# DomhnallBoyle/lip2speech-unit

Hardware: AMD Instinct MI355X
Metric: real-time factor (audio-sec/wall-sec), end-to-end lip->16kHz audio, 4s@25fps clips (higher is better)
Workload: dtype fp16; 1 GPU; e2e lip->units->wav (BASELINE configs[3]: AV-HuBERT large 24L + conformer 12x512 + multi_input HiFi-GAN), 4-s 100-frame 88x88 clips, batch 640 per GPU; clips_per_gpu=640, streams=1, clips_per_launch=640, frames_per_clip=100, hipgraph=True, input=uint8 96x96 frames resident in HBM, crop+normalise on device, enc_layers=24, conf_layers=12, parallelism=clip-parallel dp1

## Files before the change

lip2speech_unit_amd/csrc/phasegemm.hip:

```cpp
#include "l2s_common.h"
#include "tapgemm_tiles.h"
#include <cstdlib>

int l2s_phasegemm_f16_m0(const l2s_gemm_desc& d, hipStream_t st);
int l2s_phasegemm_f16_m1(const l2s_gemm_desc& d, hipStream_t st);
int l2s_phasegemm_f16_m2(const l2s_gemm_desc& d, hipStream_t st);
int l2s_phasegemm_bf16_m0(const l2s_gemm_desc& d, hipStream_t st);
int l2s_phasegemm_bf16_m1(const l2s_gemm_desc& d, hipStream_t st);
int l2s_phasegemm_bf16_m2(const l2s_gemm_desc& d, hipStream_t st);
int l2s_phasegemm_f16_m3(const l2s_gemm_desc& d, hipStream_t st);
int l2s_phasegemm_bf16_m3(const l2s_gemm_desc& d, hipStream_t st);

int l2s_phasegemm_ktab_launch(const l2s_gemm_desc& d, hipStream_t st) {
  if (d.mode != L2S_MODE_LINEAR || d.groups < 1) return L2S_EINVAL;
  const int fam = l2s::pick_epilogue(d.flags, d.act);
  if (fam != 2 && fam != l2s::L2S_EPI_G16A) return L2S_EUNSUPPORTED;
  if ((d.Cin % 64) || d.N < 256 || d.M < 256 || (d.M & 7) || (d.N & 7) || (d.lda & 7) || (d.ldc & 7) || (d.c_gstride & 63) ||
      (d.ldr & 7) || d.out_row_mul != 1 || d.out_row_add != 0)
    return L2S_EUNSUPPORTED;
  return d.dtype == L2S_F16 ? l2s_phasegemm_f16_m3(d, st) : l2s_phasegemm_bf16_m3(d, st);
}

bool l2s_phasegemm_eligible(const l2s_gemm_desc& d) {
  static const int mode = [] { const char* e = getenv("L2S_PHASEGEMM"); return e ? atoi(e) : 1; }();
  if (mode == 0) return false;
  if (d.groups > 1 || d.mode < 0 || d.mode > 2 || d.ktab) return false;
  if (d.mode == L2S_MODE_LINEAR && d.ntaps != 1) return false;
  if (d.mode == L2S_MODE_CONV1D && (d.T_out <= 0 || d.T_in <= 0)) return false;
  if (d.mode == L2S_MODE_CONV2D && (d.Ho <= 0 || d.Wo <= 0 || d.KW <= 0 || d.ntaps % d.KW)) return false;
  const int fam = l2s::pick_epilogue(d.flags, d.act);
  if (fam == l2s::L2S_EPI_ALL && !(l2s::is_x32(d.flags, d.act) && !(d.ldc & 3) && !(d.ldr & 3) && !(d.ldc2 & 3))) return false;
  static const int res_on = [] { const char* e = getenv("L2S_PHASEGEMM_RES"); return e ? atoi(e) : 1; }();
  if (!res_on && (fam == l2s::L2S_EPI_G16A || fam == l2s::L2S_EPI_G16B)) return false;
  if (fam == l2s::L2S_EPI_S32 && ((d.ldc & 3) || (d.ldr & 3))) return false;
  if ((d.Cin % 64) || d.N < 256 || d.M < 256 || (d.lda & 7)) return false;
  if (d.mode == L2S_MODE_LINEAR && ((d.M & 7) || (d.N & 7))) return false;
  if (mode == 2) return true;
  auto cdivl = [](long a, long b) { return (a + b - 1) / b; };
  const long tm = cdivl(d.M, 256);
  const long rounds_big = cdivl(tm * cdivl(d.N, 256), 256);
  if (rounds_big * ((long)d.Cin * d.ntaps / 64) < 20) return false;
  const double big = (double)rounds_big * 2.0 / 1.2;
  const double reg = (double)cdivl(tm * cdivl(d.N, 128), 256);
  return big < reg;
}

#ifdef L2S_WITH_WIDEGEMM
int l2s_widegemm_f16(const l2s_gemm_desc& d, hipStream_t st);
int l2s_widegemm_bf16(const l2s_gemm_desc& d, hipStream_t st);
static bool wide_ok(const l2s_gemm_desc& d) {
  static const int mode = [] { const char* e = getenv("L2S_WIDEGEMM"); return e ? atoi(e) : 0; }();
  if (mode == 0 || d.mode != L2S_MODE_LINEAR) return false;
  const int fam = l2s::pick_epilogue(d.flags, d.act);
  if (fam > l2s::L2S_EPI_G16A && fam != l2s::L2S_EPI_S32) return false;
  return !(d.M & 7) && !(d.N & 7);
}
#endif

int l2s_phasegemm_launch(const l2s_gemm_desc& d, hipStream_t st) {
  const bool h = d.dtype == L2S_F16;
#ifdef L2S_WITH_WIDEGEMM
  if (wide_ok(d)) return h ? l2s_widegemm_f16(d, st) : l2s_widegemm_bf16(d, st);
#endif
  switch (d.mode) {
    case L2S_MODE_LINEAR: return h ? l2s_phasegemm_f16_m0(d, st) : l2s_phasegemm_bf16_m0(d, st);
    case L2S_MODE_CONV1D: return h ? l2s_phasegemm_f16_m1(d, st) : l2s_phasegemm_bf16_m1(d, st);
    case L2S_MODE_CONV2D: return h ? l2s_phasegemm_f16_m2(d, st) : l2s_phasegemm_bf16_m2(d, st);
    default: return L2S_EINVAL;
  }
}
```

lip2speech_unit_amd/csrc/phasegemm_inst.hip:

```cpp
#include "phasegemm_kernel.h"

#define L2S_PCAT_(a, b) a##b
#define L2S_PCAT(a, b) L2S_PCAT_(a, b)
#if L2S_INST_ET == 0
using InstET = ElemF16;
#define L2S_INST_NAME L2S_PCAT(l2s_phasegemm_f16_m, L2S_INST_MODE)
#else
using InstET = ElemBF16;
#define L2S_INST_NAME L2S_PCAT(l2s_phasegemm_bf16_m, L2S_INST_MODE)
#endif

int L2S_INST_NAME(const l2s_gemm_desc& d, hipStream_t st) { return launch_phase_mode<InstET, L2S_INST_MODE>(d, st); }

#if defined(L2S_PHASE_STAMPS) && L2S_INST_ET == 0 && L2S_INST_MODE == 0
extern "C" int l2s_debug_phase_stamps(void* buf) { return phase_set_stamps(buf); }
#endif
```

lip2speech_unit_amd/csrc/phasegemm_kernel.h:

```cpp
#pragma once
#include "tapgemm_common.h"
#include <cstdlib>

using namespace l2s;

namespace {

constexpr int PBM = 256, PBN = 256, PBK = 64;
constexpr int Q_B = 128 * PBK * 2;
constexpr bool p_generic(int epi) { return epi == L2S_EPI_G16A || epi == L2S_EPI_G16B; }
constexpr int p_scr_b(int epi) { return p_generic(epi) ? 16 * 64 * 4 : 16 * (4 * 32 + 16); }
constexpr int p_smem(int epi) { return 8 * Q_B + 8 * p_scr_b(epi); }

#ifdef L2S_PHASE_STAMPS
__device__ unsigned long long* g_phase_stamps = nullptr;
#define PHSTAMP(i) { const unsigned long long now_ = __builtin_amdgcn_s_memtime(); ph_acc[i] += now_ - ph_last; ph_last = now_; }
#else
#define PHSTAMP(i)
#endif

constexpr int PG_KTAB = 3;
template <typename ET, int MODE_T, int EPI>
__global__ __launch_bounds__(512) void phasegemm_kernel(const l2s_gemm_desc p, const int tilesM, const int tilesN,
                                                        const int chunk, const int band) {
  constexpr bool KT = MODE_T == PG_KTAB;
  constexpr int MODE = KT ? (int)L2S_MODE_LINEAR : MODE_T;
  constexpr int MI = 8, NI = 4;
#ifdef L2S_NO_PAIRED
  constexpr bool PAIRED = false;
#else
  constexpr bool PAIRED = EPI <= L2S_EPI_G16A;
#endif
  extern __shared__ __attribute__((aligned(16))) uint16_t lds[];
  const int tid = threadIdx.x, lane = tid & 63;
  const int wave = __builtin_amdgcn_readfirstlane(tid >> 6);
  const int wr = wave >> 2, wc = wave & 3;
  const int K = p.Cin * p.ntaps;
  const int nk = K / PBK;
  const uint16_t* zero = reinterpret_cast<const uint16_t*>(&g_zero16);

  const int tiles_mn = tilesM * tilesN;
  const int ntiles = tiles_mn * (KT ? p.groups : 1);
  const int slot = blockIdx.x >> 3, slots = gridDim.x >> 3;
  const int lo = (blockIdx.x & 7) * chunk;
  const int hi = lo + chunk < ntiles ? lo + chunk : ntiles;
  const int my_n = (lo + slot < hi) ? (hi - lo - slot + slots - 1) / slots : 0;
  if (my_n == 0) return;
  const int total_q = my_n * nk * 4;
  auto tile_coords = [&](int i, int& m0, int& n0, int& g) {
    int l = lo + slot + i * slots;
    g = 0;
    if constexpr (KT) {
      const int per_m = p.groups * tilesN;
      const int mt = l / per_m, r = l - mt * per_m;
      g = r / tilesN;
      m0 = mt * PBM;
      n0 = (r - g * tilesN) * PBN;
      return;
    }
    const int bsz = band * tilesN;
    const int bi = l / bsz, idx = l - bi * bsz;
    const int rows = tilesM - bi * band < band ? tilesM - bi * band : band;
    const int tn = idx / rows;
    m0 = (bi * band + idx - tn * rows) * PBM;
    n0 = tn * PBN;
  };

  const int srow = lane >> 3;
  const int schunk = (lane & 7) ^ (srow & 7);
  const uint16_t* qa_ptr[2][2];
  int qa_t[2][2], qa_x[2][2];
  const uint16_t* qb_ptr[2][2];
  int run_tap = 0, run_c = 0, run_ky = 0, run_kx = 0;
  const char* sa_base[2][2] = {{nullptr, nullptr}, {nullptr, nullptr}};
  const char* sw_base[2][2] = {{nullptr, nullptr}, {nullptr, nullptr}};
  uint32_t a_lane = 0, w_lane[2] = {0, 0};
  if constexpr (MODE == L2S_MODE_LINEAR) {
    a_lane = (uint32_t)(srow * p.lda * 2 + (schunk << 4));
#pragma unroll
    for (int j = 0; j < 2; ++j) {
      const int within = 16 * (wave & 1) + 8 * j + srow;
      const int bchunk = PAIRED ? ((lane & 7) ^ paired_w_key(within)) : schunk;
      w_lane[j] = (uint32_t)(srow * K * 2 + (bchunk << 4));
    }
  }
  typedef const int32_t __attribute__((address_space(4)))* ktab_ptr_t;
  constexpr int KTN = L2S_KTAB_MAX;
  const ktab_ptr_t kt_tab = (ktab_ptr_t)(uintptr_t)p.ktab;
  ktab_ptr_t kt_row = kt_tab;
  int nk_stage = nk, kt_blk = 0, kt_win = 0;
  uint32_t kt_cur_a = 0, kt_cur_w = 0, kt_nxt_a = 0, kt_nxt_w = 0;
  const int kpb = KT ? p.Cin / PBK : 1;
  auto setup_issue = [&](int i) {
    int m0, n0, tg;
    tile_coords(i, m0, n0, tg);
    if constexpr (KT) {
      kt_row = kt_tab + tg * (2 + 2 * KTN);
      nk_stage = kt_row[0] * kpb;
      kt_blk = 0; kt_win = 0;
      kt_cur_a = (uint32_t)kt_row[2] * 2u; kt_cur_w = (uint32_t)kt_row[2 + KTN] * 2u;
      kt_nxt_a = (uint32_t)kt_row[3] * 2u; kt_nxt_w = (uint32_t)kt_row[3 + KTN] * 2u;
    }
#ifdef L2S_ABL_SAMETILE
    m0 = 0; n0 = 0;
#endif
    if constexpr (MODE == L2S_MODE_LINEAR) {
#pragma unroll
      for (int h = 0; h < 2; ++h)
#pragma unroll
        for (int j = 0; j < 2; ++j) {
          int mg = m0 + (wave >> 2) * 128 + h * 64 + 16 * (wave & 3) + 8 * j;
          mg = mg < p.M ? mg : p.M - 8;
          sa_base[h][j] = (const char*)p.A + (int64_t)mg * p.lda * 2;
          int ng = n0 + (wave >> 1) * 64 + h * 32 + 16 * (wave & 1) + 8 * j;
          ng = ng < p.N ? ng : p.N - 8;
          sw_base[h][j] = (const char*)p.W + (int64_t)ng * K * 2;
        }
      return;
    }
#pragma unroll
    for (int h = 0; h < 2; ++h)
#pragma unroll
      for (int j = 0; j < 2; ++j) {
        int m = m0 + (wave >> 2) * 128 + h * 64 + 16 * (wave & 3) + 8 * j + srow;
        m = m < p.M ? m : p.M - 1;
        qa_t[h][j] = 0; qa_x[h][j] = 0;
        if (MODE == L2S_MODE_LINEAR) {
          qa_ptr[h][j] = (const uint16_t*)p.A + (int64_t)m * p.lda + schunk * 8;
        } else if (MODE == L2S_MODE_CONV1D) {
          const int b = m / p.T_out, t = m - b * p.T_out;
          qa_ptr[h][j] = (const uint16_t*)p.A + (int64_t)b * p.T_in * p.lda + schunk * 8;
          qa_t[h][j] = t * p.stride + p.off;
        } else {
          const int hw = p.Ho * p.Wo;
          const int img = m / hw, rem = m - img * hw;
          const int oy = rem / p.Wo, ox = rem - oy * p.Wo;
          qa_ptr[h][j] = (const uint16_t*)p.A + (int64_t)img * p.Hi * p.Wi * p.lda + schunk * 8;
          qa_t[h][j] = oy * p.stride - p.pad;
          qa_x[h][j] = ox * p.stride - p.pad;
        }
        const int within = 16 * (wave & 1) + 8 * j + srow;
        int n = n0 + (wave >> 1) * 64 + h * 32 + within;
        n = n < p.N ? n : p.N - 1;
        const int bchunk = PAIRED ? ((lane & 7) ^ paired_w_key(within)) : schunk;
        qb_ptr[h][j] = (const uint16_t*)p.W + (int64_t)n * K + bchunk * 8;
      }
  };
  auto slot_off = [&](int b, int e) -> uint32_t { return (uint32_t)((b * 4 + e) * Q_B); };
  int s_i = 0, s_kt = 0, s_e = 0, s_par = 0, staged = 0;
  auto stage_one = [&](auto e_tag) {
    constexpr int E = decltype(e_tag)::value;
    const bool live = staged < total_q;
    const int k0 = s_kt * PBK;
    const int se = E >= 0 ? E : s_e;
    uint16_t* dst = lds + (slot_off(s_par, se) >> 1) + wave * 1024;
    const bool is_a = (se == 0) || (se == 3);
    const int h = (se == 2 || se == 3) ? 1 : 0;
    if constexpr (MODE == L2S_MODE_LINEAR) {
      static_assert(E >= 0, "LINEAR stages with a compile-time element");
      const uint32_t kb = (uint32_t)k0 * 2u;
      const uint32_t kba = KT ? kt_cur_a : kb, kbw = KT ? kt_cur_w : kb;
#pragma unroll
      for (int j = 0; j < 2; ++j) {
        const char* g = is_a ? sa_base[h][j] + (size_t)kba + (size_t)a_lane : sw_base[h][j] + (size_t)kbw + (size_t)w_lane[j];
#ifdef L2S_ABL_ZEROSRC
        g = (const char*)zero;
#endif
#if defined(L2S_ABL_WARMDMA)
        if (staged < 8) __builtin_amdgcn_global_load_lds((gptr_t)g, (lptr_t)(dst + j * 512), 16, 0, 0);
#elif !defined(L2S_ABL_NODMA)
        __builtin_amdgcn_global_load_lds((gptr_t)g, (lptr_t)(dst + j * 512), 16, 0, 0);
#endif
      }
      return;
    }
#pragma unroll
    for (int j = 0; j < 2; ++j) {
      const uint16_t* g;
      bool ok = live;
      if (!is_a) {
        g = qb_ptr[h][j] + k0;
      } else if (MODE == L2S_MODE_LINEAR) {
        g = qa_ptr[h][j] + k0;
      } else if (MODE == L2S_MODE_CONV1D) {
        const int st = qa_t[h][j] + run_tap * p.dil;
        ok = ok && ((unsigned)st < (unsigned)p.T_in);
        g = qa_ptr[h][j] + (st * p.lda + run_c);
      } else {
        const int iy = qa_t[h][j] + run_ky, ix = qa_x[h][j] + run_kx;
        ok = ok && ((unsigned)iy < (unsigned)p.Hi) && ((unsigned)ix < (unsigned)p.Wi);
        g = qa_ptr[h][j] + ((iy * p.Wi + ix) * p.lda + run_c);
      }
      g = ok ? g : zero;
#ifdef L2S_ABL_ZEROSRC
      g = zero;
#endif
#ifndef L2S_ABL_NODMA
      __builtin_amdgcn_global_load_lds((gptr_t)g, (lptr_t)(dst + j * 512), 16, 0, 0);
#endif
    }
  };
  auto stage_advance = [&]() {
    const bool live = staged < total_q;
    ++staged;
    if constexpr (MODE == L2S_MODE_LINEAR) {
      if (++s_e == 4) {
        s_e = 0;
        s_par ^= 1;
        if constexpr (KT) {
          if (!(s_i + 1 == my_n && s_kt + 1 == nk_stage)) {
            if (++s_kt == nk_stage) {
              s_kt = 0;
              setup_issue(++s_i);
            } else if (++kt_win == kpb) {
              kt_win = 0;
              ++kt_blk;
              kt_cur_a = kt_nxt_a; kt_cur_w = kt_nxt_w;
              const int nb = kt_blk + 1 < KTN ? kt_blk + 1 : KTN - 1;
              kt_nxt_a = (uint32_t)kt_row[2 + nb] * 2u; kt_nxt_w = (uint32_t)kt_row[2 + KTN + nb] * 2u;
            } else {
              kt_cur_a += PBK * 2; kt_cur_w += PBK * 2;
            }
          }
        } else if (staged < total_q && ++s_kt == nk) {
          s_kt = 0;
          setup_issue(++s_i);
        }
      }
      return;
    }
    if (++s_e == 4) {
      s_e = 0;
      s_par ^= 1;
      if (MODE != L2S_MODE_LINEAR) {
        run_c += PBK;
        if (run_c >= p.Cin) {
          run_c = 0;
          ++run_tap;
          if (++run_kx == p.KW) { run_kx = 0; ++run_ky; }
        }
      }
      if (live && ++s_kt == nk) {
        s_kt = 0;
        run_tap = 0; run_c = 0; run_ky = 0; run_kx = 0;
        if (++s_i < my_n) setup_issue(s_i);
      }
    }
  };

  const int lm = lane & 15, lg = lane >> 4;
  const uint32_t lds_base = (uint32_t)(uintptr_t)(lptr_t)lds;
  const uint32_t k0_off = (uint32_t)(lm * 128 + (((0 + lg) ^ (lm & 7)) << 4));
  const uint32_t k1_off = (uint32_t)(lm * 128 + (((4 + lg) ^ (lm & 7)) << 4));
  const uint32_t a_row = (uint32_t)(wr * 64) * 128;
  const uint32_t b_row = (uint32_t)(wc * 32) * 128;
  frag16 fa[4][2], fb[2][2][2];
  auto read_a = [&](uint32_t qbase) {
    const uint32_t a0 = qbase + a_row + k0_off, a1 = qbase + a_row + k1_off;
    lds_read_b128<0>(fa[0][0], a0); lds_read_b128<2048>(fa[1][0], a0); lds_read_b128<4096>(fa[2][0], a0); lds_read_b128<6144>(fa[3][0], a0);
    lds_read_b128<0>(fa[0][1], a1); lds_read_b128<2048>(fa[1][1], a1); lds_read_b128<4096>(fa[2][1], a1); lds_read_b128<6144>(fa[3][1], a1);
  };
  uint32_t bk_off[2][2];
#pragma unroll
  for (int s2 = 0; s2 < 2; ++s2)
#pragma unroll
    for (int ks = 0; ks < 2; ++ks)
      bk_off[s2][ks] = PAIRED ? paired_w_off(lm, s2, 4 * ks + lg) : (uint32_t)(s2 * 2048) + (ks ? k1_off : k0_off);
  auto read_b = [&](frag16(&f)[2][2], uint32_t qbase) {
    const uint32_t b = qbase + b_row;
    lds_read_b128<0>(f[0][0], b + bk_off[0][0]); lds_read_b128<0>(f[1][0], b + bk_off[1][0]);
    lds_read_b128<0>(f[0][1], b + bk_off[0][1]); lds_read_b128<0>(f[1][1], b + bk_off[1][1]);
  };

  f32x4_t acc[MI][NI];
#pragma unroll
  for (int i = 0; i < MI; ++i)
#pragma unroll
    for (int j = 0; j < NI; ++j) acc[i][j] = f32x4_t{0.f, 0.f, 0.f, 0.f};

  setup_issue(0);
  stage_one(std::integral_constant<int, 0>{}); stage_advance();
  stage_one(std::integral_constant<int, 1>{}); stage_advance();
  stage_one(std::integral_constant<int, 2>{}); stage_advance();
  stage_one(std::integral_constant<int, 3>{}); stage_advance();
  stage_one(std::integral_constant<int, 0>{}); stage_advance();
  stage_one(std::integral_constant<int, 1>{}); stage_advance();
  wait_vmcnt<8>();
  __builtin_amdgcn_s_barrier();
  if (wr == 1) __builtin_amdgcn_s_barrier();

  auto phase = [&](auto q_tag, const int par) {
    constexpr int Q = decltype(q_tag)::value;
#ifndef L2S_ABL_NOREAD
    if (Q == 0) { read_b(fb[0], lds_base + slot_off(par, 1)); __builtin_amdgcn_sched_barrier(0); read_a(lds_base + slot_off(par, 0)); }
    if (Q == 1) read_b(fb[1], lds_base + slot_off(par, 2));
    if (Q == 2) read_a(lds_base + slot_off(par, 3));
#endif
    stage_one(std::integral_constant<int, (Q + 2) & 3>{});
    __builtin_amdgcn_sched_barrier(0);
    wait_vmcnt<8>();
    asm volatile("" ::: "memory");
    __builtin_amdgcn_s_barrier();
    asm volatile("" ::: "memory");
    lds_wait();
    __builtin_amdgcn_s_setprio(1);
    constexpr int RH = (Q >= 2) ? 1 : 0, CH = (Q == 1 || Q == 2) ? 1 : 0;
#ifdef L2S_ABL_MFMA32
    {
      typedef __attribute__((ext_vector_type(16))) float f32x16_t;
#pragma unroll
      for (int mb = 0; mb < 2; ++mb) {
        f32x16_t c;
#pragma unroll
        for (int e = 0; e < 16; ++e) c[e] = acc[RH * 4 + mb * 2 + (e >> 3)][CH * 2 + ((e >> 2) & 1)][e & 3];
#pragma unroll
        for (int kk = 0; kk < 4; ++kk)
          c = __builtin_amdgcn_mfma_f32_32x32x16_f16(fb[CH][kk >> 1][kk & 1].h, fa[mb * 2 + (kk >> 1)][kk & 1].h, c, 0, 0, 0);
#pragma unroll
        for (int e = 0; e < 16; ++e) acc[RH * 4 + mb * 2 + (e >> 3)][CH * 2 + ((e >> 2) & 1)][e & 3] = c[e];
      }
    }
#elif !defined(L2S_ABL_NOMFMA)
#pragma unroll
    for (int i = 0; i < 4; ++i)
#pragma unroll
      for (int j = 0; j < 2; ++j) {
        acc[RH * 4 + i][CH * 2 + j] = ET::mfma(fb[CH][j][0], fa[i][0], acc[RH * 4 + i][CH * 2 + j]);
        acc[RH * 4 + i][CH * 2 + j] = ET::mfma(fb[CH][j][1], fa[i][1], acc[RH * 4 + i][CH * 2 + j]);
      }
#endif
    __builtin_amdgcn_s_setprio(0);
    __builtin_amdgcn_sched_barrier(0);
    asm volatile("" ::: "memory");
    __builtin_amdgcn_s_barrier();
    asm volatile("" ::: "memory");
    __builtin_amdgcn_sched_barrier(0);
    stage_advance();
  };

  int par = 0;
#ifdef L2S_PHASE_STAMPS
  unsigned long long ph_acc[4] = {0, 0, 0, 0};
  unsigned long long ph_last = __builtin_amdgcn_s_memtime();
  const unsigned long long ph_t0 = ph_last;
#endif
  auto nk_of = [&](int ti) -> int {
    if (ti >= my_n) return 0;
    const int l = lo + slot + ti * slots;
    const int per_m = p.groups * tilesN;
    return kt_tab[((l % per_m) / tilesN) * (2 + 2 * KTN)] * kpb;
  };
  int nk_next = KT ? nk_of(0) : nk;
  for (int ti = 0; ti < my_n; ++ti) {
    const int nk_c = nk_next;
    if constexpr (KT) nk_next = nk_of(ti + 1);
    for (int kt = 0; kt < nk_c; ++kt) {
#ifdef L2S_PHASE_STAMPS
      if (kt == 1) PHSTAMP(2)
#endif
      phase(std::integral_constant<int, 0>{}, par);
      phase(std::integral_constant<int, 1>{}, par);
      phase(std::integral_constant<int, 2>{}, par);
      phase(std::integral_constant<int, 3>{}, par);
      par ^= 1;
    }
    PHSTAMP(0)
    int m0, n0, grp;
    tile_coords(ti, m0, n0, grp);
    const uint32_t scr = lds_base + 8 * Q_B + (uint32_t)wave * p_scr_b(EPI);
    auto rowmap = [&](int m) -> int64_t { return m < p.M ? (int64_t)m * p.out_row_mul + p.out_row_add : (int64_t)-1; };
    if constexpr (EPI == L2S_EPI_X32) {
      epilogue_stream32x<ET, MI, NI>(p, acc, lane, m0 + wr * 128, n0 + wc * 64, rowmap);
    } else if constexpr (EPI == L2S_EPI_S32) {
      epilogue_direct32<ET, MI, NI>(p, acc, lane, m0 + wr * 128, n0 + wc * 64, grp, rowmap);
    } else if constexpr (PAIRED) {
      epilogue_direct16<ET, MI, NI, EPI, decltype(rowmap), NoHook, true>(p, acc, lane, m0 + wr * 128, n0 + wc * 64, grp, rowmap);
    } else if constexpr (EPI == L2S_EPI_G16A) {
      epilogue_impl<ET, MI, NI, F_G16A, true, true>(p, acc, scr, lane, m0 + wr * 128, n0 + wc * 64, grp, rowmap);
    } else if constexpr (EPI == L2S_EPI_G16B) {
      epilogue_impl<ET, MI, NI, F_G16B, true, true>(p, acc, scr, lane, m0 + wr * 128, n0 + wc * 64, grp, rowmap);
    } else {
      epilogue_fast16<ET, MI, NI, (EPI - L2S_EPI_F16) / 2, ((EPI - L2S_EPI_F16) & 1) != 0, 1>(
          p, acc, scr, lane, m0 + wr * 128, n0 + wc * 64, grp, rowmap);
    }
#pragma unroll
    for (int i = 0; i < MI; ++i)
#pragma unroll
      for (int j = 0; j < NI; ++j) acc[i][j] = f32x4_t{0.f, 0.f, 0.f, 0.f};
    PHSTAMP(1)
  }
  wait_vmcnt<0>();
#ifdef L2S_PHASE_STAMPS
  if (lane == 0 && (wave == 0 || wave == 7) && g_phase_stamps) {
    unsigned long long* o = g_phase_stamps + ((int64_t)blockIdx.x * 2 + (wave ? 1 : 0)) * 8;
    for (int i = 0; i < 3; ++i) o[i] = ph_acc[i];
    o[3] = (unsigned long long)my_n;
    o[4] = __builtin_amdgcn_s_memtime() - ph_t0;
    o[5] = (unsigned long long)nk;
  }
#endif
}

template <typename ET, int MODE, int EPI>
int launch_phase(const l2s_gemm_desc& d, hipStream_t st) {
  auto kern = phasegemm_kernel<ET, MODE, EPI>;
  static L2sSmemOptIn opt_in;
  if (int e = l2s_smem_opt_in(kern, p_smem(EPI), opt_in)) return e;
  const int tilesM = (d.M + PBM - 1) / PBM, tilesN = (d.N + PBN - 1) / PBN;
  const int ntiles = tilesM * tilesN * (MODE == PG_KTAB ? d.groups : 1);
  const int chunk = (ntiles + 7) / 8;
  const int slots = chunk < 32 ? chunk : 32;
  const double ap = (double)PBM * d.Cin * 2.0, wp = (double)PBN * d.Cin * d.ntaps * 2.0;
  auto cdivi = [](int a, int b) { return (a + b - 1) / b; };
  int band = 1;
  double best = 1e300;
  for (int b = 1; b <= tilesM; ++b) {
    const int wn = cdivi(chunk, b) < tilesN ? cdivi(chunk, b) : tilesN;
    const int an = b * cdivi(chunk, b * tilesN);
    const double fp = ap * (an < tilesM ? an : tilesM) + wp * wn;
    if (fp < best) { best = fp; band = b; }
  }
  hipLaunchKernelGGL(kern, dim3(8 * slots), dim3(512), p_smem(EPI), st, d, tilesM, tilesN, chunk, band);
  L2S_CHECK_LAUNCH();
  return L2S_OK;
}


#ifdef L2S_PHASE_STAMPS
int phase_set_stamps(void* buf) { return (int)hipMemcpyToSymbol(HIP_SYMBOL(g_phase_stamps), &buf, sizeof(buf)); }
#endif

template <typename ET, int MODE>
int launch_phase_mode(const l2s_gemm_desc& d, hipStream_t st) {
  if constexpr (MODE == PG_KTAB) {
    switch (pick_epilogue(d.flags, d.act)) {
      case 2: return launch_phase<ET, MODE, 2>(d, st);
      case L2S_EPI_G16A: return launch_phase<ET, MODE, L2S_EPI_G16A>(d, st);
      default: return L2S_EUNSUPPORTED;
    }
  } else {
    switch (pick_epilogue(d.flags, d.act)) {
      case 0: return launch_phase<ET, MODE, 0>(d, st);
      case 1: return launch_phase<ET, MODE, 1>(d, st);
      case 2: return launch_phase<ET, MODE, 2>(d, st);
      case 3: return launch_phase<ET, MODE, 3>(d, st);
      case 4: return launch_phase<ET, MODE, 4>(d, st);
      case 5: return launch_phase<ET, MODE, 5>(d, st);
      case L2S_EPI_G16A: return launch_phase<ET, MODE, L2S_EPI_G16A>(d, st);
      case L2S_EPI_G16B: return launch_phase<ET, MODE, L2S_EPI_G16B>(d, st);
      case L2S_EPI_S32: return launch_phase<ET, MODE, L2S_EPI_S32>(d, st);
      case L2S_EPI_ALL: return is_x32(d.flags, d.act) ? launch_phase<ET, MODE, L2S_EPI_X32>(d, st) : (int)L2S_EUNSUPPORTED;
      default: return L2S_EUNSUPPORTED;
    }
  }
}

}
```

lip2speech_unit_amd/csrc/tapgemm_common.h:

```cpp
#pragma once
#include "l2s_common.h"
#include "tapgemm_tiles.h"
#include <type_traits>

namespace l2s {

typedef __attribute__((address_space(1))) const void* gptr_t;
typedef __attribute__((address_space(3))) void* lptr_t;

__device__ const uint4 g_zero16 = {0u, 0u, 0u, 0u};

typedef unsigned u32x4_t __attribute__((ext_vector_type(4)));

template <int OFF>
__device__ __forceinline__ void lds_read_b128(frag16& f, uint32_t addr) {
  u32x4_t v;
  asm volatile("ds_read_b128 %0, %1 offset:%2" : "=v"(v) : "v"(addr), "n"(OFF));
  f.u = make_uint4(v.x, v.y, v.z, v.w);
}
__device__ __forceinline__ void lds_wait() {
  __builtin_amdgcn_sched_barrier(0);
  asm volatile("s_waitcnt lgkmcnt(0)" ::: "memory");
  __builtin_amdgcn_sched_barrier(0);
}
// ... 551 lines not shown
          for (int e = 0; e < 8; ++e) v[e] += rv[e];
        }
        if constexpr (ACTK == 2) {
#ifdef L2S_GELU_ERF
#pragma unroll
          for (int e = 0; e < 8; ++e) v[e] = l2s_gelu(v[e]);
#else
#pragma unroll
          for (int e = 0; e < 8; e += 2) { const f32x2_t g = l2s_gelu2(f32x2_t{v[e], v[e + 1]}); v[e] = g.x; v[e + 1] = g.y; }
#endif
        } else if constexpr (ACTK == 1) {
          if (LEAN && act == L2S_ACT_LRELU && p.act_slope > 0.f && p.act_slope <= 1.f) {
            const float s_l = p.act_slope;
#pragma unroll
            for (int e = 0; e < 8; ++e) v[e] = fmaxf(v[e], v[e] * s_l);
          } else if (LEAN && act == L2S_ACT_RELU) {
#pragma unroll
            for (int e = 0; e < 8; ++e) v[e] = fmaxf(v[e], 0.f);
          } else if (LEAN || act != L2S_ACT_NONE) {
#pragma unroll
            for (int e = 0; e < 8; ++e) v[e] = fmaxf(v[e], 0.f) + fminf(v[e], 0.f) * sj[2 * b + (e >> 2)][e & 3];
          }
        }
        if (CAN_RES && (flags & L2S_F_RES_POST)) {
#pragma unroll
          for (int e = 0; e < 8; ++e) v[e] += rv[e];
        }
        if (!keep[i]) {
#pragma unroll
          for (int e = 0; e < 8; ++e) v[e] = 0.f;
        }
        const uint4 pk = make_uint4(ET::pack2(v[0], v[1]), ET::pack2(v[2], v[3]), ET::pack2(v[4], v[5]), ET::pack2(v[6], v[7]));
        uint4 pk2 = make_uint4(0, 0, 0, 0);
        if (dual) {
          float w[8];
#pragma unroll
          for (int e = 0; e < 8; ++e) w[e] = v[e] * p.slope2;
          if (p.slope2 > 0.f && p.slope2 <= 1.f) {
#pragma unroll
            for (int e = 0; e < 8; ++e) w[e] = fmaxf(v[e], w[e]);
          } else {
#pragma unroll
            for (int e = 0; e < 8; ++e) w[e] = v[e] >= 0.f ? v[e] : w[e];
          }
          pk2 = make_uint4(ET::pack2(w[0], w[1]), ET::pack2(w[2], w[3]), ET::pack2(w[4], w[5]), ET::pack2(w[6], w[7]));
        }
        if constexpr (!FULL) {
          if (orow[i] >= 0 && okb[b]) {
            *reinterpret_cast<uint4*>((uint16_t*)p.C + (int64_t)orow[i] * p.ldc + col0 + 32 * b) = pk;
            if (dual) *reinterpret_cast<uint4*>((uint16_t*)p.C2 + (int64_t)orow[i] * p.ldc2 + col0 + 32 * b) = pk2;
          }
        } else {
          held[b & 1] = pk;
          held2[b & 1] = pk2;
          if (b & 1) {
            const bool lower = lm < 8;
            const uint4 got = dpp_row_ror8_u4(held[1]);
            const uint4 xa = lower ? held[0] : got, xb = lower ? got : held[0];
            const int hA = lm >> 3, hB = 1 - hA;
            const int cA = col0 + 32 * (b - 1) + 32 * hA, cB = col0 + 32 * (b - 1) + 32 * hB;
            const int oa = (int)rowmap(row_base + (c0 + i) * 16 + (lm & 7)), ob = (int)rowmap(row_base + (c0 + i) * 16 + 8 + (lm & 7));
            const bool okA = oa >= 0 && (hA ? okb[b] : okb[b - 1]), okB = ob >= 0 && (hB ? okb[b] : okb[b - 1]);
            if (okA) *reinterpret_cast<uint4*>((uint16_t*)p.C + (int64_t)oa * p.ldc + cA) = xa;
            if (okB) *reinterpret_cast<uint4*>((uint16_t*)p.C + (int64_t)ob * p.ldc + cB) = xb;
            if (dual) {
              const uint4 got2 = dpp_row_ror8_u4(held2[1]);
              const uint4 ya = lower ? held2[0] : got2, yb = lower ? got2 : held2[0];
              if (okA) *reinterpret_cast<uint4*>((uint16_t*)p.C2 + (int64_t)oa * p.ldc2 + cA) = ya;
              if (okB) *reinterpret_cast<uint4*>((uint16_t*)p.C2 + (int64_t)ob * p.ldc2 + cB) = yb;
            }
          }
        }
      }
      if (c0 == 0 && i == 0) after_loads();
    }
  };
  do_chunk(std::integral_constant<int, 0>{});
  if constexpr (MI > CHK) do_chunk(std::integral_constant<int, CHK>{});
  if constexpr (MI > 2 * CHK) do_chunk(std::integral_constant<int, 2 * CHK>{});
  if constexpr (MI > 3 * CHK) do_chunk(std::integral_constant<int, 3 * CHK>{});
  static_assert(MI <= 4 * CHK, "chunk list");
}

__device__ __forceinline__ f32x4_t dpp_row_ror8(f32x4_t v) {
  float r0, r1, r2, r3;
  asm volatile("s_nop 1\n\tv_mov_b32_dpp %0, %4 row_ror:8 row_mask:0xf bank_mask:0xf\n\t"
               "v_mov_b32_dpp %1, %5 row_ror:8 row_mask:0xf bank_mask:0xf\n\t"
               "v_mov_b32_dpp %2, %6 row_ror:8 row_mask:0xf bank_mask:0xf\n\t"
               "v_mov_b32_dpp %3, %7 row_ror:8 row_mask:0xf bank_mask:0xf"
               : "=&v"(r0), "=&v"(r1), "=&v"(r2), "=&v"(r3)
               : "v"(v[0]), "v"(v[1]), "v"(v[2]), "v"(v[3]));
  return f32x4_t{r0, r1, r2, r3};
}

template <typename ET, int MI, int NI, typename RowMap>
__device__ __forceinline__ void epilogue_stream32(const l2s_gemm_desc& p, f32x4_t (&acc)[MI][NI], const int lane,
                                                  const int row_base, const int ncol_base, RowMap rowmap) {
  static_assert(MI % 2 == 0 && MI >= 4 && NI % 2 == 0, "row groups are streamed in pairs, two pairs in flight; blocks in pairs");
  constexpr int NB = NI / 2;
  const int lm = lane & 15, lg = lane >> 4;
  const bool lower = lm < 8;
  const float alpha = p.alpha;
  const char* __restrict__ rbase = (const char*)p.R;
  char* __restrict__ cbase = (char*)p.C;
  f32x4_t bj[NI];
#pragma unroll
  for (int j = 0; j < NI; ++j) {
    bj[j] = f32x4_t{0.f, 0.f, 0.f, 0.f};
    if (p.bias) { const float4 q = *reinterpret_cast<const float4*>(p.bias + ncol_base + j * 16 + lg * 4); bj[j] = f32x4_t{q.x, q.y, q.z, q.w}; }
  }
  const uint32_t colA = (uint32_t)(ncol_base + 16 * (lm >> 3) + lg * 4) * 4u;
  const uint32_t colB = (uint32_t)(ncol_base + 16 * (1 - (lm >> 3)) + lg * 4) * 4u;
  const uint32_t pitch = (uint32_t)p.ldc * 4u;
  const uint32_t gstep = 16u * (uint32_t)p.out_row_mul * pitch;
  const uint32_t offA0 = (uint32_t)rowmap(row_base + (lm & 7)) * pitch + colA;
  const uint32_t offB0 = (uint32_t)rowmap(row_base + 8 + (lm & 7)) * pitch + colB;
  auto ld = [&](uint32_t off) {
    const float4 q = *reinterpret_cast<const float4*>(rbase + (size_t)off);
    return f32x4_t{q.x, q.y, q.z, q.w};
  };
  auto st = [&](uint32_t off, f32x4_t v) { *reinterpret_cast<float4*>(cbase + (size_t)off) = make_float4(v[0], v[1], v[2], v[3]); };
  auto load_pair = [&](f32x4_t (&rv)[2][NB][2], auto pr_tag) {
    constexpr int pr = decltype(pr_tag)::value;
#pragma unroll
    for (int g = 0; g < 2; ++g)
#pragma unroll
      for (int b = 0; b < NB; ++b) {
        rv[g][b][0] = ld(offA0 + (uint32_t)(2 * pr + g) * gstep + (uint32_t)(b * 128));
        rv[g][b][1] = ld(offB0 + (uint32_t)(2 * pr + g) * gstep + (uint32_t)(b * 128));
      }
  };
  auto finish_pair = [&](f32x4_t (&rv)[2][NB][2], auto pr_tag) {
    constexpr int pr = decltype(pr_tag)::value;
#pragma unroll
    for (int g = 0; g < 2; ++g)
#pragma unroll
      for (int b = 0; b < NB; ++b) {
        const int i = 2 * pr + g;
        const f32x4_t u0 = (acc[i][2 * b] + bj[2 * b]) * alpha;
        const f32x4_t u1 = (acc[i][2 * b + 1] + bj[2 * b + 1]) * alpha;
        const f32x4_t got = dpp_row_ror8(u1);
        f32x4_t xa, xb;
#pragma unroll
        for (int e = 0; e < 4; ++e) { xa[e] = lower ? u0[e] : got[e]; xb[e] = lower ? got[e] : u0[e]; }
        st(offA0 + (uint32_t)i * gstep + (uint32_t)(b * 128), xa + rv[g][b][0]);
        st(offB0 + (uint32_t)i * gstep + (uint32_t)(b * 128), xb + rv[g][b][1]);
      }
  };
  f32x4_t ra[2][NB][2], rb[2][NB][2];
  load_pair(ra, std::integral_constant<int, 0>{});
  load_pair(rb, std::integral_constant<int, 1>{});
  finish_pair(ra, std::integral_constant<int, 0>{});
  if constexpr (MI > 4) load_pair(ra, std::integral_constant<int, 2>{});
  finish_pair(rb, std::integral_constant<int, 1>{});
  if constexpr (MI > 6) load_pair(rb, std::integral_constant<int, 3>{});
  if constexpr (MI > 4) finish_pair(ra, std::integral_constant<int, 2>{});
  if constexpr (MI > 6) finish_pair(rb, std::integral_constant<int, 3>{});
  static_assert(MI <= 8, "row group pairs");
}

template <typename ET, int MI, int NI, typename RowMap>
__device__ __forceinline__ void epilogue_stream32x(const l2s_gemm_desc& p, f32x4_t (&acc)[MI][NI], const int lane,
                                                   const int row_base, const int ncol_base, RowMap rowmap) {
  static_assert(MI % 2 == 0, "row groups are streamed in pairs");
  const int lm = lane & 15, lg = lane >> 4;
  const int flags = p.flags;
// ... 181 lines not shown
```

Before: 13620 audio-sec/wall-sec.

## Add rolling-drain phase GEMM that overlaps tile epilogue with next tile's mainloop

Adds a ROLL variant of the persistent phase GEMM for plain linear layers with an f16 epilogue (none, relu/lrelu or gelu), full 256-tiles and no residual. The previous tile's output rows are stored during the first k-tiles of the next tile, and the bias is prefetched into LDS during the last k-tiles. The first k-tile zero-initialises the accumulators inside the MFMA instead of running a separate clear. The aim is to hide the epilogue store and bias latency behind MFMA work, at the cost of more scheduling complexity, hand-tuned vmcnt values and register pressure. The variant is on by default through an environment variable.

```diff
diff --git a/lip2speech_unit_amd/csrc/phasegemm.hip b/lip2speech_unit_amd/csrc/phasegemm.hip
--- a/lip2speech_unit_amd/csrc/phasegemm.hip
+++ b/lip2speech_unit_amd/csrc/phasegemm.hip
@@ -1,5 +1,6 @@
 #include "l2s_common.h"
 #include "tapgemm_tiles.h"
+#include <atomic>
 #include <cstdlib>
 
 int l2s_phasegemm_f16_m0(const l2s_gemm_desc& d, hipStream_t st);
@@ -10,6 +11,8 @@
 int l2s_phasegemm_bf16_m2(const l2s_gemm_desc& d, hipStream_t st);
 int l2s_phasegemm_f16_m3(const l2s_gemm_desc& d, hipStream_t st);
 int l2s_phasegemm_bf16_m3(const l2s_gemm_desc& d, hipStream_t st);
+int l2s_phasegemm_f16_m4(const l2s_gemm_desc& d, hipStream_t st);
+int l2s_phasegemm_bf16_m4(const l2s_gemm_desc& d, hipStream_t st);
 
 int l2s_phasegemm_ktab_launch(const l2s_gemm_desc& d, hipStream_t st) {
   if (d.mode != L2S_MODE_LINEAR || d.groups < 1) return L2S_EINVAL;
@@ -57,11 +60,30 @@
 }
 #endif
 
+static bool roll_ok(const l2s_gemm_desc& d) {
+  static const int roll_on = [] { const char* e = getenv("L2S_PHASEGEMM_ROLL"); return e ? atoi(e) : 1; }();
+  if (!roll_on || d.mode != L2S_MODE_LINEAR || d.ktab || d.groups > 1 || d.ntaps != 1) return false;
+  const int fam = l2s::pick_epilogue(d.flags, d.act);
+  if (fam != l2s::L2S_EPI_F16 && fam != l2s::L2S_EPI_F16 + 2 && fam != l2s::L2S_EPI_F16 + 4) return false;
+  if (fam == l2s::L2S_EPI_F16 + 2 && !(d.act == L2S_ACT_RELU || (d.act == L2S_ACT_LRELU && d.act_slope > 0.f && d.act_slope <= 1.f)))
+    return false;
+  if ((d.M % 256) || (d.N % 256) || (d.Cin % 64) || d.Cin / 64 < 4) return false;
+  if (d.out_row_mul != 1 || d.out_row_add != 0 || d.R || (d.ldc & 7)) return false;
+  return true;
+}
+
+static std::atomic<long> g_roll_launches{0};
+extern "C" long l2s_debug_phasegemm_roll_launches() { return g_roll_launches.load(); }
+
 int l2s_phasegemm_launch(const l2s_gemm_desc& d, hipStream_t st) {
   const bool h = d.dtype == L2S_F16;
 #ifdef L2S_WITH_WIDEGEMM
   if (wide_ok(d)) return h ? l2s_widegemm_f16(d, st) : l2s_widegemm_bf16(d, st);
 #endif
+  if (roll_ok(d)) {
+    ++g_roll_launches;
+    return h ? l2s_phasegemm_f16_m4(d, st) : l2s_phasegemm_bf16_m4(d, st);
+  }
   switch (d.mode) {
     case L2S_MODE_LINEAR: return h ? l2s_phasegemm_f16_m0(d, st) : l2s_phasegemm_bf16_m0(d, st);
     case L2S_MODE_CONV1D: return h ? l2s_phasegemm_f16_m1(d, st) : l2s_phasegemm_bf16_m1(d, st);
diff --git a/lip2speech_unit_amd/csrc/phasegemm_inst.hip b/lip2speech_unit_amd/csrc/phasegemm_inst.hip
--- a/lip2speech_unit_amd/csrc/phasegemm_inst.hip
+++ b/lip2speech_unit_amd/csrc/phasegemm_inst.hip
@@ -10,8 +10,15 @@
 #define L2S_INST_NAME L2S_PCAT(l2s_phasegemm_bf16_m, L2S_INST_MODE)
 #endif
 
+#if L2S_INST_MODE == 4
+int L2S_INST_NAME(const l2s_gemm_desc& d, hipStream_t st) { return launch_phase_roll<InstET>(d, st); }
+#else
 int L2S_INST_NAME(const l2s_gemm_desc& d, hipStream_t st) { return launch_phase_mode<InstET, L2S_INST_MODE>(d, st); }
+#endif
 
 #if defined(L2S_PHASE_STAMPS) && L2S_INST_ET == 0 && L2S_INST_MODE == 0
 extern "C" int l2s_debug_phase_stamps(void* buf) { return phase_set_stamps(buf); }
 #endif
+#if defined(L2S_PHASE_STAMPS) && L2S_INST_ET == 0 && L2S_INST_MODE == 4
+extern "C" int l2s_debug_phase_stamps_roll(void* buf) { return phase_set_stamps(buf); }
+#endif
diff --git a/lip2speech_unit_amd/csrc/phasegemm_kernel.h b/lip2speech_unit_amd/csrc/phasegemm_kernel.h
--- a/lip2speech_unit_amd/csrc/phasegemm_kernel.h
+++ b/lip2speech_unit_amd/csrc/phasegemm_kernel.h
@@ -20,7 +20,18 @@
 #endif
 
 constexpr int PG_KTAB = 3;
-template <typename ET, int MODE_T, int EPI>
+template <int N> using ic = std::integral_constant<int, N>;
+
+constexpr int DR_NONE = -1, DR_BIAS = 4;
+
+template <int N>
+__device__ __forceinline__ void lgkm_wait_pin4(f32x4_t (&b)[4]) {
+  __builtin_amdgcn_sched_barrier(0);
+  asm volatile("s_waitcnt lgkmcnt(%4)" : "+v"(b[0]), "+v"(b[1]), "+v"(b[2]), "+v"(b[3]) : "n"(N) : "memory");
+  __builtin_amdgcn_sched_barrier(0);
+}
+
+template <typename ET, int MODE_T, int EPI, bool ROLL = false>
 __global__ __launch_bounds__(512) void phasegemm_kernel(const l2s_gemm_desc p, const int tilesM, const int tilesN,
                                                         const int chunk, const int band) {
   constexpr bool KT = MODE_T == PG_KTAB;
@@ -31,6 +42,7 @@
 #else
   constexpr bool PAIRED = EPI <= L2S_EPI_G16A;
 #endif
+  static_assert(!ROLL || (MODE_T == L2S_MODE_LINEAR && PAIRED && (EPI == 0 || EPI == 2 || EPI == 4)), "rolling drain: see above");
   extern __shared__ __attribute__((aligned(16))) uint16_t lds[];
   const int tid = threadIdx.x, lane = tid & 63;
   const int wave = __builtin_amdgcn_readfirstlane(tid >> 6);
@@ -47,7 +59,7 @@
   const int my_n = (lo + slot < hi) ? (hi - lo - slot + slots - 1) / slots : 0;
   if (my_n == 0) return;
   const int total_q = my_n * nk * 4;
-  auto tile_coords = [&](int i, int& m0, int& n0, int& g) {
+  auto tile_coords = [&](int i, int& m0, int& n0, int& g) __attribute__((always_inline)) {
     int l = lo + slot + i * slots;
     g = 0;
     if constexpr (KT) {
@@ -91,7 +103,7 @@
   int nk_stage = nk, kt_blk = 0, kt_win = 0;
   uint32_t kt_cur_a = 0, kt_cur_w = 0, kt_nxt_a = 0, kt_nxt_w = 0;
   const int kpb = KT ? p.Cin / PBK : 1;
-  auto setup_issue = [&](int i) {
+  auto setup_issue = [&](int i) __attribute__((always_inline)) {
     int m0, n0, tg;
     tile_coords(i, m0, n0, tg);
     if constexpr (KT) {
@@ -146,9 +158,9 @@
         qb_ptr[h][j] = (const uint16_t*)p.W + (int64_t)n * K + bchunk * 8;
       }
   };
-  auto slot_off = [&](int b, int e) -> uint32_t { return (uint32_t)((b * 4 + e) * Q_B); };
+  auto slot_off = [&](int b, int e) __attribute__((always_inline)) -> uint32_t { return (uint32_t)((b * 4 + e) * Q_B); };
   int s_i = 0, s_kt = 0, s_e = 0, s_par = 0, staged = 0;
-  auto stage_one = [&](auto e_tag) {
+  auto stage_one = [&](auto e_tag) __attribute__((always_inline)) {
     constexpr int E = decltype(e_tag)::value;
     const bool live = staged < total_q;
     const int k0 = s_kt * PBK;
@@ -200,7 +212,7 @@
 #endif
     }
   };
-  auto stage_advance = [&]() {
+  auto stage_advance = [&]() __attribute__((always_inline)) {
     const bool live = staged < total_q;
     ++staged;
     if constexpr (MODE == L2S_MODE_LINEAR) {
@@ -255,7 +267,7 @@
   const uint32_t a_row = (uint32_t)(wr * 64) * 128;
   const uint32_t b_row = (uint32_t)(wc * 32) * 128;
   frag16 fa[4][2], fb[2][2][2];
-  auto read_a = [&](uint32_t qbase) {
+  auto read_a = [&](uint32_t qbase) __attribute__((always_inline)) {
     const uint32_t a0 = qbase + a_row + k0_off, a1 = qbase + a_row + k1_off;
     lds_read_b128<0>(fa[0][0], a0); lds_read_b128<2048>(fa[1][0], a0); lds_read_b128<4096>(fa[2][0], a0); lds_read_b128<6144>(fa[3][0], a0);
     lds_read_b128<0>(fa[0][1], a1); lds_read_b128<2048>(fa[1][1], a1); lds_read_b128<4096>(fa[2][1], a1); lds_read_b128<6144>(fa[3][1], a1);
@@ -266,7 +278,7 @@
 #pragma unroll
     for (int ks = 0; ks < 2; ++ks)
       bk_off[s2][ks] = PAIRED ? paired_w_off(lm, s2, 4 * ks + lg) : (uint32_t)(s2 * 2048) + (ks ? k1_off : k0_off);
-  auto read_b = [&](frag16(&f)[2][2], uint32_t qbase) {
+  auto read_b = [&](frag16(&f)[2][2], uint32_t qbase) __attribute__((always_inline)) {
     const uint32_t b = qbase + b_row;
     lds_read_b128<0>(f[0][0], b + bk_off[0][0]); lds_read_b128<0>(f[1][0], b + bk_off[1][0]);
     lds_read_b128<0>(f[0][1], b + bk_off[0][1]); lds_read_b128<0>(f[1][1], b + bk_off[1][1]);
@@ -285,20 +297,55 @@
   stage_one(std::integral_constant<int, 3>{}); stage_advance();
   stage_one(std::integral_constant<int, 0>{}); stage_advance();
   stage_one(std::integral_constant<int, 1>{}); stage_advance();
-  wait_vmcnt<8>();
+  wait_vmcnt<ROLL ? 0 : 8>();
   __builtin_amdgcn_s_barrier();
   if (wr == 1) __builtin_amdgcn_s_barrier();
 
-  auto phase = [&](auto q_tag, const int par) {
+  char* dr_base = nullptr;
+  const char* dr_bias = reinterpret_cast<const char*>(zero);
+  const uint32_t dr_scr = lds_base + 8 * Q_B + (uint32_t)wave * p_scr_b(EPI);
+  auto dr_lane = [&]() __attribute__((always_inline)) -> int { int l = lane; asm volatile("" : "+v"(l)); return l; };
+  auto drain_step = [&](auto dr_tag) __attribute__((always_inline)) {
+    constexpr int RG0 = 2 * decltype(dr_tag)::value;
+    f32x4_t dr_bj[4];
+    const int dl = dr_lane();
+    const uint32_t dr_brd = dr_scr + (uint32_t)(dl >> 4) * 32u;
+    uint32_t dr_offA, dr_offB;
+    direct16_lane_offs(dl, p.ldc, dr_offA, dr_offB);
+    dr_bj[0] = lds_read_f4<0>(dr_brd); dr_bj[1] = lds_read_f4<16>(dr_brd);
+    dr_bj[2] = lds_read_f4<128>(dr_brd); dr_bj[3] = lds_read_f4<144>(dr_brd);
+    lgkm_wait_pin4<0>(dr_bj);
+    const uint32_t rg_b = (uint32_t)(16 * p.ldc * 2);
+    direct16_rowgroup<ET, EPI>(p, acc[RG0], dr_bj, dr_base + (size_t)(RG0 * rg_b), dr_offA, dr_offB, dl);
+    __builtin_amdgcn_sched_barrier(0);
+    direct16_rowgroup<ET, EPI>(p, acc[RG0 + 1], dr_bj, dr_base + (size_t)((RG0 + 1) * rg_b), dr_offA, dr_offB, dl);
+    __builtin_amdgcn_sched_barrier(0);
+  };
+  auto phase_x = [&](auto q_tag, const int par, auto vm_tag, auto dr_tag, auto z_tag) __attribute__((always_inline)) {
+    constexpr bool Z = decltype(z_tag)::value != 0;
     constexpr int Q = decltype(q_tag)::value;
+    constexpr int VM = decltype(vm_tag)::value, DR = decltype(dr_tag)::value;
+    constexpr bool DRAIN = ROLL && DR >= 0 && DR < 4;
+    static_assert(ROLL || (VM == 8 && DR == DR_NONE), "only the rolling variant changes a phase");
+    auto frag_reads = [&]() __attribute__((always_inline)) {
 #ifndef L2S_ABL_NOREAD
-    if (Q == 0) { read_b(fb[0], lds_base + slot_off(par, 1)); __builtin_amdgcn_sched_barrier(0); read_a(lds_base + slot_off(par, 0)); }
-    if (Q == 1) read_b(fb[1], lds_base + slot_off(par, 2));
-    if (Q == 2) read_a(lds_base + slot_off(par, 3));
-#endif
-    stage_one(std::integral_constant<int, (Q + 2) & 3>{});
+      if (Q == 0) { read_b(fb[0], lds_base + slot_off(par, 1)); __builtin_amdgcn_sched_barrier(0); read_a(lds_base + slot_off(par, 0)); }
+      if (Q == 1) read_b(fb[1], lds_base + slot_off(par, 2));
+      if (Q == 2) read_a(lds_base + slot_off(par, 3));
+#endif
+    };
+    if constexpr (!DRAIN) {
+      frag_reads();
+      stage_one(std::integral_constant<int, (Q + 2) & 3>{});
+      if constexpr (ROLL && DR == DR_BIAS)
+        __builtin_amdgcn_global_load_lds((gptr_t)(dr_bias + (size_t)(p.bias ? (uint32_t)dr_lane() * 4u : 0u)), (lptr_t)((char*)lds + 8 * Q_B + wave * p_scr_b(EPI)), 4, 0, 0);
+    } else {
+      stage_one(std::integral_constant<int, (Q + 2) & 3>{});
+      drain_step(dr_tag);
+      frag_reads();
+    }
     __builtin_amdgcn_sched_barrier(0);
-    wait_vmcnt<8>();
+    wait_vmcnt<VM>();
     asm volatile("" ::: "memory");
     __builtin_amdgcn_s_barrier();
     asm volatile("" ::: "memory");
@@ -325,7 +372,7 @@
     for (int i = 0; i < 4; ++i)
 #pragma unroll
       for (int j = 0; j < 2; ++j) {
-        acc[RH * 4 + i][CH * 2 + j] = ET::mfma(fb[CH][j][0], fa[i][0], acc[RH * 4 + i][CH * 2 + j]);
+        acc[RH * 4 + i][CH * 2 + j] = ET::mfma(fb[CH][j][0], fa[i][0], Z ? f32x4_t{0.f, 0.f, 0.f, 0.f} : acc[RH * 4 + i][CH * 2 + j]);
         acc[RH * 4 + i][CH * 2 + j] = ET::mfma(fb[CH][j][1], fa[i][1], acc[RH * 4 + i][CH * 2 + j]);
       }
 #endif
@@ -337,6 +384,7 @@
     __builtin_amdgcn_sched_barrier(0);
     stage_advance();
   };
+  auto phase = [&](auto q_tag, const int par) { phase_x(q_tag, par, ic<8>{}, ic<DR_NONE>{}, ic<0>{}); };
 
   int par = 0;
 #ifdef L2S_PHASE_STAMPS
@@ -351,6 +399,42 @@
     return kt_tab[((l % per_m) / tilesN) * (2 + 2 * KTN)] * kpb;
   };
   int nk_next = KT ? nk_of(0) : nk;
+  if constexpr (ROLL) {
+    auto ktile = [&](auto z, auto v0, auto d0, auto v1, auto d1, auto v2, auto d2, auto v3, auto d3) __attribute__((always_inline)) {
+      phase_x(ic<0>{}, par, v0, d0, z);
+      phase_x(ic<1>{}, par, v1, d1, z);
+      phase_x(ic<2>{}, par, v2, d2, z);
+      phase_x(ic<3>{}, par, v3, d3, z);
+      par ^= 1;
+    };
+    auto ktile_plain = [&](auto z) __attribute__((always_inline)) {
+      ktile(z, ic<8>{}, ic<DR_NONE>{}, ic<8>{}, ic<DR_NONE>{}, ic<8>{}, ic<DR_NONE>{}, ic<8>{}, ic<DR_NONE>{});
+    };
+    {
+      int m0, n0, grp;
+      tile_coords(0, m0, n0, grp);
+      dr_base = (char*)p.C + ((int64_t)(m0 + wr * 128) * p.ldc + n0 + wc * 64) * 2;
+    }
+    PHSTAMP(3)
+    for (int ti = 0; ti < my_n; ++ti) {
+      if (ti) { PHSTAMP(2) }
+      ktile(ic<1>{}, ic<20>{}, ic<2>{}, ic<24>{}, ic<3>{}, ic<24>{}, ic<DR_NONE>{}, ic<20>{}, ic<DR_NONE>{});
+      ktile(ic<0>{}, ic<16>{}, ic<DR_NONE>{}, ic<12>{}, ic<DR_NONE>{}, ic<8>{}, ic<DR_NONE>{}, ic<8>{}, ic<DR_NONE>{});
+      PHSTAMP(2)
+      for (int kt = 2; kt < nk - 2; ++kt) ktile_plain(ic<0>{});
+      PHSTAMP(0)
+      int m0, n0, grp;
+      tile_coords(ti, m0, n0, grp);
+      dr_base = (char*)p.C + ((int64_t)(m0 + wr * 128) * p.ldc + n0 + wc * 64) * 2;
+      if (p.bias) dr_bias = reinterpret_cast<const char*>(p.bias + n0 + wc * 64);
+      ktile(ic<0>{}, ic<9>{}, ic<DR_BIAS>{}, ic<9>{}, ic<DR_NONE>{}, ic<9>{}, ic<DR_NONE>{}, ic<9>{}, ic<DR_NONE>{});
+      ktile(ic<0>{}, ic<9>{}, ic<DR_NONE>{}, ic<8>{}, ic<DR_NONE>{}, ic<12>{}, ic<0>{}, ic<16>{}, ic<1>{});
+    }
+    PHSTAMP(2)
+    drain_step(ic<2>{});
+    drain_step(ic<3>{});
+    PHSTAMP(1)
+  } else
   for (int ti = 0; ti < my_n; ++ti) {
     const int nk_c = nk_next;
     if constexpr (KT) nk_next = nk_of(ti + 1);
@@ -401,9 +485,9 @@
 #endif
 }
 
-template <typename ET, int MODE, int EPI>
+template <typename ET, int MODE, int EPI, bool ROLL = false>
 int launch_phase(const l2s_gemm_desc& d, hipStream_t st) {
-  auto kern = phasegemm_kernel<ET, MODE, EPI>;
+  auto kern = phasegemm_kernel<ET, MODE, EPI, ROLL>;
   static L2sSmemOptIn opt_in;
   if (int e = l2s_smem_opt_in(kern, p_smem(EPI), opt_in)) return e;
   const int tilesM = (d.M + PBM - 1) / PBM, tilesN = (d.N + PBN - 1) / PBN;
@@ -430,6 +514,16 @@
 int phase_set_stamps(void* buf) { return (int)hipMemcpyToSymbol(HIP_SYMBOL(g_phase_stamps), &buf, sizeof(buf)); }
 #endif
 
+template <typename ET>
+int launch_phase_roll(const l2s_gemm_desc& d, hipStream_t st) {
+  switch (pick_epilogue(d.flags, d.act)) {
+    case 0: return launch_phase<ET, L2S_MODE_LINEAR, 0, true>(d, st);
+    case 2: return launch_phase<ET, L2S_MODE_LINEAR, 2, true>(d, st);
+    case 4: return launch_phase<ET, L2S_MODE_LINEAR, 4, true>(d, st);
+    default: return L2S_EUNSUPPORTED;
+  }
+}
+
 template <typename ET, int MODE>
 int launch_phase_mode(const l2s_gemm_desc& d, hipStream_t st) {
   if constexpr (MODE == PG_KTAB) {
diff --git a/lip2speech_unit_amd/csrc/tapgemm_common.h b/lip2speech_unit_amd/csrc/tapgemm_common.h
--- a/lip2speech_unit_amd/csrc/tapgemm_common.h
+++ b/lip2speech_unit_amd/csrc/tapgemm_common.h
@@ -657,6 +657,55 @@
   static_assert(MI <= 4 * CHK, "chunk list");
 }
 
+__device__ __forceinline__ void direct16_lane_offs(const int lane, const int ldc, uint32_t& offA, uint32_t& offB) {
+  const int lm = lane & 15, lg = lane >> 4, hA = lm >> 3;
+  offA = (uint32_t)(((lm & 7) * ldc + 8 * lg + 32 * hA) * 2);
+  offB = (uint32_t)(((8 + (lm & 7)) * ldc + 8 * lg + 32 * (1 - hA)) * 2);
+}
+template <typename ET, int EPI>
+__device__ __forceinline__ void direct16_rowgroup(const l2s_gemm_desc& p, const f32x4_t (&a)[4], const f32x4_t (&bj)[4], char* cbase,
+                                                  const uint32_t offA, const uint32_t offB, const int lane) {
+  static_assert(EPI == L2S_EPI_F16 || EPI == L2S_EPI_F16 + 2 || EPI == L2S_EPI_F16 + 4, "lean families without mask");
+  constexpr int ACTK = (EPI - L2S_EPI_F16) / 2;
+  const float alpha = p.alpha;
+  const int act = p.act;
+  uint4 held[2];
+#pragma unroll
+  for (int b = 0; b < 2; ++b) {
+    float v[8];
+#pragma unroll
+    for (int e = 0; e < 8; ++e) v[e] = a[2 * b + (e >> 2)][e & 3] + bj[2 * b + (e >> 2)][e & 3];
+    if (alpha != 1.f) {
+#pragma unroll
+      for (int e = 0; e < 8; ++e) v[e] *= alpha;
+    }
+    if constexpr (ACTK == 2) {
+#ifdef L2S_GELU_ERF
+#pragma unroll
+      for (int e = 0; e < 8; ++e) v[e] = l2s_gelu(v[e]);
+#else
+#pragma unroll
+      for (int e = 0; e < 8; e += 2) { const f32x2_t g = l2s_gelu2(f32x2_t{v[e], v[e + 1]}); v[e] = g.x; v[e + 1] = g.y; }
+#endif
+    } else if constexpr (ACTK == 1) {
+      if (act == L2S_ACT_LRELU && p.act_slope > 0.f && p.act_slope <= 1.f) {
+        const float s_l = p.act_slope;
+#pragma unroll
+        for (int e = 0; e < 8; ++e) v[e] = fmaxf(v[e], v[e] * s_l);
+      } else {
+#pragma unroll
+        for (int e = 0; e < 8; ++e) v[e] = fmaxf(v[e], 0.f);
+      }
+    }
+    held[b] = make_uint4(ET::pack2(v[0], v[1]), ET::pack2(v[2], v[3]), ET::pack2(v[4], v[5]), ET::pack2(v[6], v[7]));
+  }
+  const bool lower = (lane & 15) < 8;
+  const uint4 got = dpp_row_ror8_u4(held[1]);
+  const uint4 xa = lower ? held[0] : got, xb = lower ? got : held[0];
+  *reinterpret_cast<uint4*>(cbase + offA) = xa;
+  *reinterpret_cast<uint4*>(cbase + offB) = xb;
+}
+
 __device__ __forceinline__ f32x4_t dpp_row_ror8(f32x4_t v) {
   float r0, r1, r2, r3;
   asm volatile("s_nop 1\n\tv_mov_b32_dpp %0, %4 row_ror:8 row_mask:0xf bank_mask:0xf\n\t"
```

Result: no change. 13750 audio-sec/wall-sec (median of 6 runs) (+0.9%).
